# rbarile17/kelpie

Measured on AMD Instinct MI355X. Metric: candidate explanations evaluated/sec (incl. post-train) + rank-delta match rate, higher is better.
Workload: dtype bf16x3 (fp32-emulated)

## Files before the change

### kelpie_amd/csrc/kp_api.hip

```cpp
#include <cmath>
#include <cstdio>
#include <cstdlib>

#include "kp_common.hpp"
#include "kp_trace_check.hpp"

int cx_pick_db(int dim);

static thread_local std::string g_tls_err;

template <class F>
static int guarded(kp_ctx* c, F&& f) {
  try {
    f();
    if (c) c->err.clear();
    return KP_OK;
  } catch (const KpError& e) {
    if (c) c->err = e.msg;
    g_tls_err = e.msg;
    return e.code;
  } catch (const std::bad_alloc&) {
    if (c) c->err = "host out of memory";
    g_tls_err = "host out of memory";
    return KP_ENOMEM;
// ... 83 lines not shown
      KP_REQUIRE(m->model != KP_MODEL_COMPLEX || m->dim % 2 == 0, "ComplEx: row width must be even ([Re | Im])");
      int db = cx_pick_db(m->dim);
      KP_REQUIRE(db > 0, "row width > 400 not supported yet for ComplEx / ConvE");
      c->dp = 16 * db;
    } else if (m->model == KP_MODEL_DISTMULT) {
      int db = cx_pick_db(m->dim);
      if (db <= 0) throw KpError{KP_ENOTSUP, "DistMult: row width > 400 not supported"};
      c->dp = 16 * db;
    } else {
      c->dp = round_up(m->dim, 16);
    }
    c->attn_mode = 1;
    if (const char* a = std::getenv("KP_ATTN")) c->attn_mode = std::strcmp(a, "f32") == 0 ? 0 : 1;
    c->cv_fused = 1;
    if (const char* a = std::getenv("KP_CV_FUSED")) c->cv_fused = std::atoi(a) != 0;
    c->cv_shared = 1;
    if (const char* a = std::getenv("KP_CV_SHARED")) c->cv_shared = std::atoi(a) != 0;
    if (const char* a = std::getenv("KP_CV_RANK")) c->cv_rank64 = std::strcmp(a, "f32") != 0;
    if (const char* a = std::getenv("KP_CV_DX")) c->cv_dx_block = std::strcmp(a, "block") == 0;
    if (const char* a = std::getenv("KP_TE_RANK")) c->te_rank64 = std::strcmp(a, "f32") != 0;
    if (const char* a = std::getenv("KP_ATTN_PART"))
      c->attn_part = std::strcmp(a, "streamk") == 0 ? 1 : std::strcmp(a, "ranges") == 0 ? 2 : 0;
    if (const char* a = std::getenv("KP_ATTN_RANGES")) c->attn_ranges = std::max(0, std::min(16, std::atoi(a)));
    KP_HIP(hipStreamCreateWithFlags(&c->stream, hipStreamNonBlocking));
    {
      hipMemPool_t pool = device_pool(device);
      for (DevBuf* d : c->buffers()) {
        d->s = c->stream;
        d->pool = pool;
      }
    }
    KP_HIP(hipEventCreate(&c->ev0));
    KP_HIP(hipEventCreate(&c->ev1));
    upload_padded(c, &c->dE, m->entity, m->n_ent, m->dim, c->dp);
    upload_padded(c, &c->dR, m->relation, m->n_rel2, m->dim, c->dp);
    if (m->model == KP_MODEL_CONVE) {
      KP_REQUIRE(m->conv_w && m->conv_b && m->fc_w && m->fc_b && m->bn_alpha && m->bn_beta,
                 "ConvE: missing frozen layers");
      KP_REQUIRE(m->dim % 20 == 0 && m->dim / 20 >= 3, "ConvE: dim must be 20*h with h >= 3");
      c->hidden = 32 * 38 * (m->dim / 20 - 2);
      upload_plain(&c->d_conv_w, m->conv_w, 32 * 9);
      upload_plain(&c->d_conv_b, m->conv_b, 32);
      upload_plain(&c->d_fc_w, m->fc_w, (size_t)m->dim * c->hidden);
      upload_plain(&c->d_fc_b, m->fc_b, m->dim);
      upload_plain(&c->d_bn_a, m->bn_alpha, 1 + 32 + m->dim);
      upload_plain(&c->d_bn_b, m->bn_beta, 1 + 32 + m->dim);
// ... 315 lines not shown
```

### kelpie_amd/csrc/kp_attn3.hpp

```cpp
#pragma once
#include <type_traits>

#include "kp_attn.hpp"

#ifdef KP_ATTN3_STAMPS
#ifndef KP_DIAGNOSTIC_BUILD
#error "KP_ATTN3_STAMPS is a diagnostic build (make diag / tools/attn_micro.sh)"
#endif
__device__ unsigned long long g_attn3_stamps[8];
#define KP3_STAMP(v) v = __builtin_amdgcn_s_memtime()
#define KP3_ACC(i, a, b) st_acc[i] += (b) - (a)
#else
#define KP3_STAMP(v) (void)0
#define KP3_ACC(i, a, b) (void)0
#endif

#ifdef KP_ATTN3_CLOCK
#ifndef KP_DIAGNOSTIC_BUILD
#error "KP_ATTN3_CLOCK is a diagnostic build (tools/attn_micro.sh)"
#endif
__device__ unsigned long long g_attn3_clock[4096][4];
#endif

#ifndef KP_O_AHEAD
#define KP_O_AHEAD 1
#endif
#ifndef KP_S_AHEAD
#define KP_S_AHEAD 1
#endif
static_assert(KP_S_AHEAD >= 1 && KP_S_AHEAD <= 2, "KP_S_AHEAD: 1..2 (lgkmcnt holds at most 15)");
#if (defined(KP_DIAG_NO_S) || defined(KP_DIAG_NO_O) || defined(KP_ATTN_NODMA) || defined(KP_DIAG_DMA_LGKM0) || \
     defined(KP_DMA_SPREAD_ALL) || defined(KP_DIAG_S4) || defined(KP_DIAG_DMA_VM0) || defined(KP_DIAG_M0SAVE) || defined(KP_DIAG_NO_OSTORE) || defined(KP_DIAG_EARLY_EXIT) || defined(KP_DIAG_O_HALF) || defined(KP_DIAG_S_HALF) || defined(KP_DIAG_XTILE_W)) && \
// ... 145 lines not shown
  return c;
}

template <int DP>
__global__ void kp_split3_table(const float* __restrict__ E, int n_ent, uint8_t* __restrict__ out) {
  const long long i = (long long)blockIdx.x * blockDim.x + threadIdx.x;
  if (i >= (long long)n_ent * (DP / 2)) return;
  const int e = (int)(i / (DP / 2)), d = 2 * (int)(i % (DP / 2));
  __bf16 h[2], m[2], l[2];
  split3(E[(size_t)e * DP + d], h[0], m[0], l[0]);
  split3(E[(size_t)e * DP + d + 1], h[1], m[1], l[1]);
  __bf16* row = reinterpret_cast<__bf16*>(out + (size_t)e * split3_row_bytes(DP));
  row[d] = h[0];
  row[d + 1] = h[1];
  row[DP + d] = m[0];
  row[DP + d + 1] = m[1];
  row[2 * DP + d] = l[0];
  row[2 * DP + d + 1] = l[1];
}

template <int DB, int MODE>
constexpr int attn3_min_wgs() { return (MODE == ATT_BCE_O && 2 * attn3_lds_bytes(DB) <= 163840) ? 2 : 1; }

template <int DB, int MODE>
__global__ __launch_bounds__(256, (attn3_min_wgs<DB, MODE>())) void kp_attn3(const uint8_t* __restrict__ E3, int n_ent,
                                                   const float* __restrict__ Qpre, int nq, AttnWork wk,
                                                   float* __restrict__ out_m, float* __restrict__ out_l,
                                                   float* __restrict__ out_O, const float* __restrict__ qscale,
                                                   float ylo, const double* __restrict__ colpre) {
  constexpr bool WITH_O = MODE != ATT_SOFTMAX;
  constexpr int DP = 16 * DB;
  constexpr bool ASM = attn3_asm(DB);
  constexpr bool ILV = ASM && KP_ILV;
  constexpr int NK = DP / 32;
  constexpr int TAIL = (DP % 32) / 16;
  constexpr int KT = 32;
  constexpr int PART_B = 2 * DP;
  constexpr int ROW_B = split3_row_bytes(DP);
  constexpr bool BUFDMA = attn3_bufdma(DB);
  constexpr int PIECES = attn3_buf_pieces(DB);
  constexpr int BUF_B = 1024 * PIECES;
  extern __shared__ __attribute__((aligned(16))) uint8_t lds3[];

  const int tid = threadIdx.x;
#ifdef KP_DIAG_EARLY_EXIT
  if (ylo != 12345.f) return;
#endif
  if constexpr (KP_ATTN_PRIO > 0) __builtin_amdgcn_s_setprio(KP_ATTN_PRIO);
  const int lane = tid & 63;
  const int w = __builtin_amdgcn_readfirstlane(tid >> 6);
  const int g = lane >> 4, c = lane & 15;
  int key_begin = 0, key_end = 0;
  const uint32_t lds0 = (uint32_t)(uintptr_t)(__attribute__((address_space(3))) uint8_t*)lds3;
#ifdef KP_ATTN3_STAMPS
  unsigned long long st0 = 0, st1 = 0, st2 = 0, st3 = 0, st4 = 0;
  unsigned long long st_acc[5] = {0, 0, 0, 0, 0};
#endif

  const __amdgpu_buffer_rsrc_t e3rsrc = __builtin_amdgcn_make_buffer_rsrc(
      const_cast<uint8_t*>(E3), (short)0, (int)((n_ent + 31) / 32 * 32 * ROW_B + 1024), 0x00020000);
#if KP_O_SC1
  const __amdgpu_buffer_rsrc_t orsrc =
      __builtin_amdgcn_make_buffer_rsrc(out_O, (short)0, 0x7FFFFFFF, 0x00020000);
#endif
  auto bdma = [&](int tile, int buf, int p) {
    __builtin_amdgcn_raw_ptr_buffer_load_lds(
        e3rsrc, (__attribute__((address_space(3))) void*)(uintptr_t)(lds0 + (uint32_t)(buf * BUF_B + 1024 * p)), 16,
        16 * lane, (key_begin + tile * KT) * ROW_B + 1024 * p, 0, 0);
  };
  typedef int i32x4_t __attribute__((ext_vector_type(4)));
  const i32x4_t e3rs = {(int)(uint32_t)(uintptr_t)E3,
                        (int)(uint32_t)((uintptr_t)E3 >> 32) & 0xFFFF,
                        (int)((n_ent + 31) / 32 * 32 * ROW_B + 1024), 0x00020000};
  auto dma_group = [&](int tile, int buf, int g) {
    const int pb = w * ((PIECES + 3) / 4) + 4 * g;
    const uint32_t m0v = (uint32_t)__builtin_amdgcn_readfirstlane((int)(lds0 + (uint32_t)(buf * BUF_B + 1024 * pb)));
    const uint32_t so = (uint32_t)__builtin_amdgcn_readfirstlane((key_begin + tile * KT) * ROW_B + 1024 * pb);
    const int nleft = (PIECES + 3) / 4 - 4 * g;
    uint32_t keep;
// ... 82 lines not shown
  for (;;) {
    int qt, kt0, kt1, part;
    bool fill_rest;
    if (wk.ranges) {
      if (unit >= n_units) break;
      qt = unit % QT;
      part = unit / QT;
      kt0 = (int)((long long)part * wk.ktq / wk.ranges);
      kt1 = (int)((long long)(part + 1) * wk.ktq / wk.ranges);
      fill_rest = false;
      unit += (int)gridDim.x;
    } else {
      if (it >= it_end) break;
      qt = (int)(it / wk.ktq);
      kt0 = (int)(it - (long long)qt * wk.ktq);
      kt1 = (int)min((long long)wk.ktq, (long long)kt0 + (it_end - it));
      part = (int)blockIdx.x - (int)(((long long)qt * wk.ktq) / wk.per_wg);
      fill_rest = kt1 == wk.ktq;
      it += kt1 - kt0;
    }
    key_begin = kt0 * KT;
    key_end = min(n_ent, kt1 * KT);
    const int ntiles = kt1 - kt0;
    const int q = qt * 64 + 16 * w + c;
    const bool valid = q < nq;
    bf16x8 qb[NK > 0 ? NK : 1][3];
    bf16x4 qt4[3];
    float gsc = 0.f;
    if (MODE == ATT_BCE_O) gsc = valid ? qscale[q] : 0.f;
    {
      const float* qp = Qpre + (size_t)(valid ? q : 0) * DP;
#pragma unroll
      for (int s = 0; s < NK; ++s) {
        const float4 v0 = *reinterpret_cast<const float4*>(qp + 32 * s + 8 * g);
        const float4 v1 = *reinterpret_cast<const float4*>(qp + 32 * s + 8 * g + 4);
        const float f[8] = {v0.x, v0.y, v0.z, v0.w, v1.x, v1.y, v1.z, v1.w};
#pragma unroll
        for (int j = 0; j < 8; ++j) {
          __bf16 h, m, l;
          split3(valid ? f[j] : 0.f, h, m, l);
          qb[s][0][j] = h;
          qb[s][1][j] = m;
          qb[s][2][j] = l;
        }
      }
      if (TAIL) {
        const float4 v0 = *reinterpret_cast<const float4*>(qp + 32 * NK + 4 * g);
        const float f[4] = {v0.x, v0.y, v0.z, v0.w};
#pragma unroll
        for (int j = 0; j < 4; ++j) {
          __bf16 h, m, l;
          split3(valid ? f[j] : 0.f, h, m, l);
          qt4[0][j] = h;
          qt4[1][j] = m;
          qt4[2][j] = l;
        }
      }
    }
    f32x4 O[WITH_O ? DB : 1];
    float m_ref = kNegInf, l_run = 0.f;
    float csh = 0.f;

    for (int pass = 0; pass < 2; ++pass) {
#pragma unroll
      for (int j = 0; j < (WITH_O ? DB : 1); ++j) O[j] = (f32x4){0.f, 0.f, 0.f, 0.f};
      l_run = 0.f;
      float m_seen = kNegInf;
      if (ntiles > 0) issue(0, 0);
      asm volatile("s_waitcnt vmcnt(0)" ::: "memory");
      __syncthreads();
#ifdef KP_DIAG_XTILE_W
      float scp[2][4] = {{0.f, 0.f, 0.f, 0.f}, {0.f, 0.f, 0.f, 0.f}};
      float pwn[8] = {0.f, 0.f, 0.f, 0.f, 0.f, 0.f, 0.f, 0.f};
      float lacc = 0.f;
      bf16x8 pbn[3];
      float dtmp[8], htmp[8];
      auto wpiece = [&](int q) {
        if (q < 24) {
          const int j = q / 3, st = q % 3;
          if (st == 0) {
            dtmp[j] = scp[j >> 2][j & 3] - m_ref;
            m_seen = fmaxf(m_seen, scp[j >> 2][j & 3]);
          } else if (st == 1) {
            pwn[j] = __expf(dtmp[j]);
          } else {
            pwn[j] = __fsub_rn(pwn[j], csh);
            lacc += pwn[j];
          }
        } else if (q < 48) {
          const int j = (q - 24) / 3, st = (q - 24) % 3;
          if (st == 0) {
            const __bf16 h = (__bf16)pwn[j];
            pbn[0][j] = h;
// ... 333 lines not shown
        }
        KP3_STAMP(st3);
        asm volatile("s_waitcnt vmcnt(0)" ::: "memory");
        __syncthreads();
        KP3_STAMP(st4);
        KP3_ACC(0, st0, st1);
        KP3_ACC(1, st1, st2);
        KP3_ACC(2, st2, st3);
        KP3_ACC(3, st3, st4);
#ifdef KP_ATTN3_STAMPS
        st_acc[4] += 1;
#endif
      }
      if (MODE == ATT_BCE_O) break;
      float mq = fmaxf(m_seen, __shfl_xor(m_seen, 16, 64));
      mq = fmaxf(mq, __shfl_xor(mq, 32, 64));
#if defined(KP_DIAG_NO_S) || defined(KP_DIAG_NO_O)
      break;
#endif
      if (pass == 1 || !__syncthreads_or(mq > m_ref + kMargin)) break;
      m_ref = mq;
    }

    float l_tot = l_run + __shfl_xor(l_run, 16, 64);
    l_tot += __shfl_xor(l_tot, 32, 64);
    if (ntiles > 0) {
      l_tot = __fmaf_rn(csh, (float)(key_end - key_begin), l_tot);
      if (WITH_O) {
        const double* p0 = colpre + (size_t)kt0 * DP;
        const double* p1 = colpre + (size_t)kt1 * DP;
#pragma unroll
        for (int m = 0; m < DB; ++m) {
          const int d = 16 * m + 4 * g;
          const double2 a0 = *reinterpret_cast<const double2*>(p0 + d), a1 = *reinterpret_cast<const double2*>(p0 + d + 2);
          const double2 b0 = *reinterpret_cast<const double2*>(p1 + d), b1 = *reinterpret_cast<const double2*>(p1 + d + 2);
          O[m][0] = __fmaf_rn(csh, (float)(b0.x - a0.x), O[m][0]);
          O[m][1] = __fmaf_rn(csh, (float)(b0.y - a0.y), O[m][1]);
          O[m][2] = __fmaf_rn(csh, (float)(b1.x - a1.x), O[m][2]);
          O[m][3] = __fmaf_rn(csh, (float)(b1.y - a1.y), O[m][3]);
        }
      }
    }
    if (valid) {
      const size_t o = (size_t)part * nq + q;
      if (g == 0 && MODE != ATT_BCE_O) {
        out_m[o] = m_ref;
        out_l[o] = l_tot;
      }
#ifdef KP_DIAG_NO_OSTORE
      if (false) {
#else
// ... 7 lines not shown
          __builtin_amdgcn_raw_buffer_store_b128(__builtin_bit_cast(u32x4_t, O[m]), orsrc,
                                                 (int)((o * DP + 16 * m + 4 * g) * sizeof(float)), 0, 16);
#elif KP_O_NT
          __builtin_nontemporal_store(O[m], reinterpret_cast<f32x4*>(dst + 16 * m + 4 * g));
#else
          *reinterpret_cast<float4*>(dst + 16 * m + 4 * g) = make_float4(O[m][0], O[m][1], O[m][2], O[m][3]);
#endif
        }
      }
    }
    if (fill_rest && valid) {
      for (int pp = part + 1; pp < wk.n_parts; ++pp) {
        const size_t o = (size_t)pp * nq + q;
        if (g == 0 && MODE != ATT_BCE_O) {
          out_m[o] = kNegInf;
          out_l[o] = 0.f;
        }
        if (WITH_O) {
          float* dst = out_O + o * DP;
          for (int d = 4 * g; d < DP; d += 16) *reinterpret_cast<float4*>(dst + d) = make_float4(0.f, 0.f, 0.f, 0.f);
        }
      }
    }
  }
#ifdef KP_ATTN3_STAMPS
  if (lane == 0)
    for (int i = 0; i < 5; ++i) atomicAdd(&g_attn3_stamps[i], st_acc[i]);
#endif
#ifdef KP_ATTN3_CLOCK
  {
    unsigned long long ck_t1, ck_r1;
    asm volatile("s_waitcnt vmcnt(0)\n\ts_memtime %0\n\ts_memrealtime %1\n\ts_waitcnt lgkmcnt(0)"
                 : "=s"(ck_t1), "=s"(ck_r1)::"memory");
    if (tid == 0 && blockIdx.x < 4096) {
      g_attn3_clock[blockIdx.x][0] = ck_t0;
      g_attn3_clock[blockIdx.x][1] = ck_r0;
      g_attn3_clock[blockIdx.x][2] = ck_t1;
      g_attn3_clock[blockIdx.x][3] = ck_r1;
    }
  }
#endif
}

template <int DB>
const uint8_t* split3_image(kp_ctx* c) {
  constexpr int DP = 16 * DB;
  KP_REQUIRE(c->dp == DP, "attn3: table stride mismatch");
  if (!c->e3_ready) {
    const size_t n_pad = (size_t)(c->n_ent + 31) / 32 * 32;
    const size_t bytes = n_pad * split3_row_bytes(DP) + 1024;
// ... 23 lines not shown
  if (d >= DP) return;
  double s = 0.0;
  pre[d] = 0.0;
  for (int t = 0; t < ntiles; ++t) {
    s += ts[(size_t)t * DP + d];
    pre[(size_t)(t + 1) * DP + d] = s;
  }
}
template <int DB>
const double* tile_prefix(kp_ctx* c) {
  constexpr int DP = 16 * DB;
  if (!c->e3pre_ready) {
    const int ntiles = (c->n_ent + 31) / 32;
    double* ts = reinterpret_cast<double*>(c->e3ts.ensure(sizeof(double) * (size_t)ntiles * DP));
    double* pre = reinterpret_cast<double*>(c->e3pre.ensure(sizeof(double) * (size_t)(ntiles + 1) * DP));
    hipLaunchKernelGGL((kp_tile_sums<DP>), dim3((unsigned)ntiles), dim3((DP + 63) / 64 * 64), 0, c->stream, c->dE,
                       c->n_ent, ts);
    KP_HIP(hipGetLastError());
    hipLaunchKernelGGL((kp_tile_prefix<DP>), dim3((DP + 63) / 64), dim3(64), 0, c->stream, ts, ntiles, pre);
    KP_HIP(hipGetLastError());
    c->e3pre_ready = true;
  }
  return c->e3pre.as<double>();
}

template <int DB, int MODE = ATT_SOFTMAX_O>
int attn3_wpc(kp_ctx* c) {
  static_assert(MODE == ATT_SOFTMAX_O || MODE == ATT_BCE_O, "attn3_wpc: the launched O mode");
  int& slot = c->attn3_wpc[MODE == ATT_BCE_O ? 1 : 0];
  if (slot <= 0) {
    int n = 0;
    KP_HIP(hipOccupancyMaxActiveBlocksPerMultiprocessor(&n, kp_attn3<DB, MODE>, 256, attn3_lds_bytes(DB)));
    slot = std::max(1, n);
  }
  return slot;
}

#define KP_DB_CASE(N, DB_MIN, ...)   \
  case N:                            \
    if constexpr (N >= (DB_MIN)) {   \
      constexpr int DB = N;          \
      __VA_ARGS__;                   \
    }                                \
    break;
#define KP_DB_DISPATCH(DBV, DB_MIN, MSG, ...)      \
  switch ((DBV) >= (DB_MIN) ? (DBV) : -1) {        \
// ... 7 lines not shown
    default: throw KpError{KP_ENOTSUP, MSG};       \
  }

#ifndef KP_CV_ATTN_INFLIGHT
#define KP_CV_ATTN_INFLIGHT 0
#endif

inline AttnPlan attn_plan_ctx(const kp_ctx* c, int nq, int n_ent, int slots, bool inflight_ok) {
  if (c->attn_mode != 1) return attn_plan(nq, n_ent, slots);
  return attn_plan_select(c->attn_part, inflight_ok ? c->attn_inflight : 1, c->attn_ranges, nq, n_ent, slots);
}

inline void attn_plan_note(kp_ctx* c, const AttnPlan& p, int nq, bool inflight_ok) {
  if (nq < c->attn_last.nq) return;
  c->attn_last.nq = nq;
  c->attn_last.inflight = (c->attn_mode == 1 && inflight_ok) ? c->attn_inflight : 1;
  c->attn_last.ranges = p.wk.ranges;
  c->attn_last.n_parts = p.wk.n_parts;
  c->attn_last.n_wg = p.n_wg;
}

template <int DB, int MODE>
void launch_attn3(kp_ctx* c, int n_ent, const float* Q, int nq, const AttnPlan& plan, float* m, float* l, float* O,
                  const float* qscale, float ylo) {
  KP_REQUIRE(n_ent == c->n_ent, "attn3: key count differs from the table's (tile prefix sums)");
  KP_REQUIRE((long long)(n_ent + 31) / 32 * 32 * split3_row_bytes(16 * DB) + 1024 < (1LL << 31),
             "attn3: table too large for the 32-bit buffer descriptor of the split image");
  const uint8_t* E3 = split3_image<DB>(c);
  const double* pre = tile_prefix<DB>(c);
  hipLaunchKernelGGL((kp_attn3<DB, MODE>), dim3(plan.n_wg), dim3(256), attn3_lds_bytes(DB), c->stream, E3, n_ent, Q,
                     nq, plan.wk, m, l, O, qscale, ylo, pre);
  KP_HIP(hipGetLastError());
}

}
```

### kelpie_amd/csrc/kp_common.hpp

```cpp
#pragma once

#include <hip/hip_runtime.h>

#include <algorithm>
#include <array>
#include <cstdint>
#include <cstring>
#include <mutex>
#include <string>
#include <tuple>
#include <utility>
#include <vector>

#include "../../include/kelpie_hip.h"

typedef float f32x4 __attribute__((ext_vector_type(4)));

#define KP_WAVE 64

struct KpError {
  int code;
  std::string msg;
};

// ... 75 lines not shown
  DevBuf cand_key, cand_col;
  DevBuf top_ids, top_scores;
  DevBuf p_trip, p_po, p_filt_off, p_filt;
  DevBuf p_target, p_rank;
  DevBuf p_q64, p_t64, p_bits;
  auto all() {
    return std::array{&pred,     &po,       &filt_off, &filt,       &target,     &rank,   &q64,
                      &t64,      &scores,   &bits,     &cand_key,   &cand_col,   &top_ids, &top_scores,
                      &p_trip,   &p_po,     &p_filt_off, &p_filt,   &p_target,   &p_rank, &p_q64,
                      &p_t64,    &p_bits};
  }
};
KP_WS_COMPLETE(RankWs);

struct ComplexWs {
  DevBuf x, s1, s2;
  DevBuf plans, queries, targets;
  DevBuf pairs, acts;
  DevBuf stepq, stept;
  DevBuf contrib;
  DevBuf tsum, qpair, lsef;
  DevBuf am, al, ao;
  DevBuf qs;
  DevBuf score_q, score_out;
  DevBuf tr_term, tr_fe, tr_fr, tr_off, tr_loss;
  auto all() {
    return std::array{&x, &s1, &s2, &plans, &queries, &targets, &pairs, &acts, &stepq, &stept, &contrib,
                      &tsum, &qpair, &lsef, &am, &al, &ao, &qs, &score_q, &score_out, &tr_term, &tr_fe, &tr_fr,
                      &tr_off, &tr_loss};
  }
};
KP_WS_COMPLETE(ComplexWs);

struct TranseWs {
  DevBuf x;
  DevBuf slots, rows, rng;
  DevBuf order;
  DevBuf heads, rels;
  DevBuf tr_off, tr_loss;
  auto all() { return std::array{&x, &slots, &rows, &rng, &order, &heads, &rels, &tr_off, &tr_loss}; }
};
KP_WS_COMPLETE(TranseWs);

struct ConveWs {
  DevBuf x, s1, s2;
  DevBuf kinst, finst, acts;
  DevBuf tails;
  DevBuf keep_bits;
  DevBuf fcf, fpairs;
  DevBuf flat;
  DevBuf slab;
// ... 40 lines not shown
  int n_ent = 0, n_rel2 = 0, dim = 0, dp = 0;
  int hidden = 0;
  float* dE = nullptr;
  float* dR = nullptr;
  float* d_conv_w = nullptr;
  float* d_conv_b = nullptr;
  float* d_fc_w = nullptr;
  float* d_fc_wt = nullptr;
  float* d_fc_b = nullptr;
  float* d_bn_a = nullptr;
  float* d_bn_b = nullptr;
  std::vector<float> hE;
  RankWs rank;
  ComplexWs cx;
  TranseWs te;
  ConveWs cv;
  std::string err;
  Timing timing;
  bool time_hot = true;
  int attn_mode = 0;
  int attn_part = 0;
  int attn_inflight = 1;
  int attn_ranges = 0;
  struct AttnLast {
    int nq = -1, inflight = 1, ranges = 0, n_parts = 0, n_wg = 0;
  } attn_last;
  bool e3_ready = false;
  bool e3pre_ready = false;
  bool eT_ready = false;
  int cv_fused = 1;
  int cv_rank64 = 1;
  int cv_dx_block = 0;
  int te_norm = 2;
  int te_rank64 = 1;
  bool cvf_ready = false;
  int cv_shared = 1;
  bool cv_shared_ready = false;
  int attn3_wpc[2] = {0, 0};
  kp_train_state* train = nullptr;
  kp_cv_train* cvtrain = nullptr;
  std::vector<hipEvent_t> evpool;
  std::vector<std::pair<double, double>> hot_pairs;
  std::vector<double> hot_iv;
  std::vector<DevBuf*> buffers() {
    std::vector<DevBuf*> v;
    auto add = [&v](auto list) { v.insert(v.end(), list.begin(), list.end()); };
// ... 122 lines not shown
```

### kelpie_amd/csrc/kp_complex.hip

```cpp
#include <algorithm>
#include <cstdio>
#include <cstdlib>
#include <cmath>

#include "kp_attn.hpp"
#include "kp_attn3.hpp"
#include "kp_cx_plan.hpp"
#include "kp_posttrain.hpp"

namespace {
using namespace kpattn;

__device__ __forceinline__ double cx_q64(const float* __restrict__ lhs, const float* __restrict__ rel, int d,
                                         int half) {
  if (d < half) return (double)lhs[d] * (double)rel[d] - (double)lhs[d + half] * (double)rel[d + half];
  if (d < 2 * half) {
    const int i = d - half;
    return (double)lhs[i] * (double)rel[d] + (double)lhs[d] * (double)rel[i];
  }
  return 0.0;
}

struct CxProd {
  static constexpr int G = 2;
// ... 23 lines not shown

struct DmProd {
  static constexpr int G = 1;
  static constexpr const char* name = "DistMult";
  static int extent(int dim) { return dim; }
  static __device__ __forceinline__ float q(const float* __restrict__ lhs, const float* __restrict__ rel, int d,
                                            int w) {
    return d < w ? __fmul_rn(lhs[d], rel[d]) : 0.f;
  }
  static __device__ __forceinline__ double q64(const float* __restrict__ lhs, const float* __restrict__ rel, int d,
                                               int w) {
    return d < w ? (double)lhs[d] * (double)rel[d] : 0.0;
  }
  static __device__ __forceinline__ float mod(const float* xv) { return fabsf(xv[0]); }
  static __device__ __forceinline__ double mod64(const float* xv) { return fabs((double)xv[0]); }
  static __device__ __forceinline__ void emit(float* __restrict__ out, int i, int w, const double* xv,
                                              const double* rv, const double* dv, double cf) {
    const double q = xv[0] * rv[0];
    out[i] = (float)(dv[0] * rv[0] + cf * q);
  }
};

template <class Prod>
__global__ void kp_cx_qpair(const float* __restrict__ E, const float* __restrict__ R, int dp, int half,
                            const int2* __restrict__ pairs, int n_pairs, float* __restrict__ out) {
  int p = blockIdx.x;
  if (p >= n_pairs) return;
  int2 hr = pairs[p];
  const float* lhs = E + (size_t)hr.x * dp;
  const float* rel = R + (size_t)hr.y * dp;
  for (int d = threadIdx.x; d < dp; d += blockDim.x) out[(size_t)p * dp + d] = Prod::q(lhs, rel, d, half);
}

__global__ void kp_cx_lse_merge(int npairs, int n_split, const float* __restrict__ am, const float* __restrict__ al,
                                float* __restrict__ lsef) {
  const int p = blockIdx.x * blockDim.x + threadIdx.x;
  if (p >= npairs) return;
  float mm = kNegInf;
  for (int s = 0; s < n_split; ++s) mm = fmaxf(mm, am[(size_t)s * npairs + p]);
  double ll = 0.0;
  for (int s = 0; s < n_split; ++s) {
    const float ms = am[(size_t)s * npairs + p];
    if (ms != kNegInf) ll += (double)al[(size_t)s * npairs + p] * exp((double)ms - (double)mm);
  }
  lsef[p] = (float)((double)mm + log(ll));
}

__global__ void kp_cx_tsum(const float* __restrict__ E, int dp, const CxQuery* __restrict__ pq, int nq,
                           const int32_t* __restrict__ targets, float* __restrict__ tsum) {
  int q = blockIdx.x;
  if (q >= nq) return;
  CxQuery Q = pq[q];
  for (int d = threadIdx.x; d < dp; d += blockDim.x) {
    float acc = 0.f;
// ... 381 lines not shown
      const float* eo = E + (size_t)o * DP;
      for (int d = 0; d < DP; ++d) t = __fma_rn(q[d], (double)eo[d], t);
    } else {
      t = z;
    }
    kcol64[s] = z;
    t64[s] = t;
  }
}

template <class Prod>
__global__ void kp_cx_scoreq(const float* __restrict__ E, const float* __restrict__ R, int dp, int half,
                             const int32_t* __restrict__ heads, const int32_t* __restrict__ rels, int n,
                             float* __restrict__ Q) {
  int s = blockIdx.x;
  if (s >= n) return;
  const float* lhs = E + (size_t)heads[s] * dp;
  const float* rel = R + (size_t)rels[s] * dp;
  for (int d = threadIdx.x; d < dp; d += blockDim.x) Q[(size_t)s * dp + d] = Prod::q(lhs, rel, d, half);
}

template <int DP, class Prod>
__global__ void kp_cx_stepq(const float* __restrict__ X, const float* __restrict__ R, int half,
                            const int4* __restrict__ stepq, int nq, float* __restrict__ Q) {
  const int j = blockIdx.x;
  if (j >= nq) return;
  const int4 sq = stepq[j];
  const float* x = X + (size_t)sq.x * DP;
  const float* rel = R + (size_t)sq.y * DP;
  for (int d = threadIdx.x; d < DP; d += blockDim.x) Q[(size_t)j * DP + d] = Prod::q(x, rel, d, half);
}

template <int DB, class Prod>
void launch_stepq(kp_ctx* c, const int4* stepq, const float* X, int nq, float* Q) {
  if (nq <= 0) return;
  hipLaunchKernelGGL((kp_cx_stepq<16 * DB, Prod>), dim3(nq), dim3(64), 0, c->stream, X, c->dR, Prod::extent(c->dim), stepq,
                     nq, Q);
  KP_HIP(hipGetLastError());
}

template <int DB>
int attn_slots_db(kp_ctx* c) {
  if (c->attn_mode == 1) return c->n_cu * attn3_wpc<DB>(c);
  return c->n_cu * (DB <= 13 ? 2 : 1);
}

template <int DB>
void launch_attn(kp_ctx* c, bool with_o, const float* Q, int nq, const AttnPlan& plan, float* m, float* l,
                 float* O) {
  if (nq <= 0) return;
  if (c->attn_mode == 1) {
    if (with_o)
      launch_attn3<DB, ATT_SOFTMAX_O>(c, c->n_ent, Q, nq, plan, m, l, O, nullptr, 0.f);
    else
      launch_attn3<DB, ATT_SOFTMAX>(c, c->n_ent, Q, nq, plan, m, l, O, nullptr, 0.f);
    return;
  }
  const size_t shm = attn_lds_bytes(DB);
  if (with_o)
    hipLaunchKernelGGL((kp_attn<DB, ATT_SOFTMAX_O>), dim3(plan.n_wg), dim3(256), shm, c->stream, c->dE, c->n_ent, Q,
                       nq, plan.wk, m, l, O, nullptr, 0.f);
  else
    hipLaunchKernelGGL((kp_attn<DB, ATT_SOFTMAX>), dim3(plan.n_wg), dim3(256), shm, c->stream, c->dE, c->n_ent, Q,
                       nq, plan.wk, m, l, O, nullptr, 0.f);
  KP_HIP(hipGetLastError());
}

struct CxTraceDev {
  double *term = nullptr, *freg_e = nullptr, *freg_r = nullptr;
  const int32_t* targets = nullptr;
  const int2* pairs = nullptr;
  int32_t* off = nullptr;
  float* loss = nullptr;
  int total = 0;
};

template <int DB, class Prod>
void launch_update(kp_ctx* c, int n_act, const int4* act, const CxPlan* plans, const CxQuery* pq,
// ... 53 lines not shown
  opt.one_minus_b1 = (float)(1.0 - (double)hp->beta1);
  opt.one_minus_b2 = (float)(1.0 - (double)hp->beta2);
  opt.reg_w = hp->reg_weight;
  KP_REQUIRE(hp->reg_kind == KP_REG_N3 || hp->reg_kind == KP_REG_N2, who + ": unknown regulariser");
  opt.reg_n2 = hp->reg_kind == KP_REG_N2;
  return opt;
}

struct CxDev {
  float *X, *S1, *S2;
  CxPlan* plans;
  CxQuery* pq;
  int32_t* tg;
  int2* pairs;
  int4 *acts, *stepq, *stept;
  float *contrib, *tsum, *qpair, *lsef;
  Rank64Dev r64;
  int32_t* pred;
  RankDev rk;
  ProbeDev probes;
  CxTraceDev trace;
  float *am = nullptr, *al = nullptr, *ao = nullptr, *qs = nullptr;
  std::vector<AttnPlan> step_plan;
};

static_assert(sizeof(CxI2) == sizeof(int2) && alignof(CxI2) == alignof(int2), "CxI2 is int2");
static_assert(sizeof(CxI4) == sizeof(int4) && alignof(CxI4) == alignof(int4), "CxI4 is int4");
inline const int2* as_dev(const CxI2* p) { return reinterpret_cast<const int2*>(p); }
inline const int4* as_dev(const CxI4* p) { return reinterpret_cast<const int4*>(p); }

CxDev cx_workspaces(kp_ctx* c, const kp_batch* bt, const TopkOut& tk, const CxStepPlan& sp, std::vector<float>& xp) {
  const int ns = bt->n_slots, DP = c->dp;
  CxDev d;
  d.X = upload_x0(c, c->cx.x, bt, xp);
  d.S1 = reinterpret_cast<float*>(c->cx.s1.ensure(sizeof(float) * (size_t)ns * DP));
  d.S2 = reinterpret_cast<float*>(c->cx.s2.ensure(sizeof(float) * (size_t)ns * DP));
  KP_HIP(hipMemsetAsync(d.S1, 0, sizeof(float) * (size_t)ns * DP, c->stream));
  KP_HIP(hipMemsetAsync(d.S2, 0, sizeof(float) * (size_t)ns * DP, c->stream));
  d.plans = upload(c, c->cx.plans, sp.plans.data(), sp.plans.size());
  d.pq = upload(c, c->cx.queries, sp.pqs.data(), sp.pqs.size());
  d.tg = upload(c, c->cx.targets, sp.targets.data(), sp.targets.size());
  d.pairs = upload(c, c->cx.pairs, as_dev(sp.pairs.data()), sp.pairs.size());
  d.acts = upload(c, c->cx.acts, as_dev(sp.acts.data()), sp.acts.size());
  d.stepq = upload(c, c->cx.stepq, as_dev(sp.stepq.data()), sp.stepq.size());
  d.stept = upload(c, c->cx.stept, as_dev(sp.stept.data()), sp.stept.size());
  d.contrib = reinterpret_cast<float*>(c->cx.contrib.ensure(sizeof(float) * (size_t)std::max(1, sp.max_items) * DP));
// ... 35 lines not shown
                       reg_n2, d.trace.freg_e);
    KP_HIP(hipGetLastError());
    hipLaunchKernelGGL(kp_cx_rowreg<Prod>, dim3((c->n_rel2 + 3) / 4), dim3(256), 0, c->stream, c->dR, c->n_rel2, DP,
                       half, reg_n2, d.trace.freg_r);
    KP_HIP(hipGetLastError());
  }
  int slots_attn = 0;
  CX_DISPATCH(DBV, slots_attn = attn_slots_db<DB>(c));
  const AttnPlan plan_pairs = attn_plan_ctx(c, std::max(npairs, 1), c->n_ent, slots_attn, true);
  const int split_pairs = plan_pairs.wk.n_parts;
  size_t att_rows = (size_t)std::max(npairs, 1) * split_pairs;
  d.step_plan.resize(sp.T);
  c->attn_last = {};
  for (int t = 0; t < sp.T; ++t) {
    const int nq = sp.q_off[t + 1] - sp.q_off[t];
    d.step_plan[t] = attn_plan_ctx(c, std::max(nq, 1), c->n_ent, slots_attn, true);
    if (nq > 0) attn_plan_note(c, d.step_plan[t], nq, true);
    att_rows = std::max(att_rows, (size_t)nq * d.step_plan[t].wk.n_parts);
  }
  d.am = reinterpret_cast<float*>(c->cx.am.ensure(sizeof(float) * att_rows));
  d.al = reinterpret_cast<float*>(c->cx.al.ensure(sizeof(float) * att_rows));
  d.ao = reinterpret_cast<float*>(c->cx.ao.ensure(sizeof(float) * att_rows * DP));
  d.qs = reinterpret_cast<float*>(c->cx.qs.ensure(sizeof(float) * (size_t)std::max(sp.max_nq, 1) * DP));
  if (npairs > 0) {
    hipLaunchKernelGGL(kp_cx_qpair<Prod>, dim3(npairs), dim3(128), 0, c->stream, c->dE, c->dR, DP, Prod::extent(c->dim),
                       d.pairs, npairs, d.qpair);
    KP_HIP(hipGetLastError());
    CX_DISPATCH(DBV, launch_attn<DB>(c, false, d.qpair, npairs, plan_pairs, d.am, d.al, nullptr));
    hipLaunchKernelGGL(kp_cx_lse_merge, dim3((npairs + 255) / 256), dim3(256), 0, c->stream, npairs, split_pairs, d.am,
                       d.al, d.lsef);
    KP_HIP(hipGetLastError());
  }
}

template <class Prod>
int64_t cx_step_loop(kp_ctx* c, const kp_hp* hp, const CxStepPlan& sp, const CxDev& d, CxOpt opt, double* t_steps) {
  const int DBV = c->dp / 16, T = sp.T;
  int64_t hot_launches = 0;
  c->hot_pairs.clear();
  c->hot_iv.clear();
  for (int t = 0; t < T; ++t) {
    const int nq = sp.q_off[t + 1] - sp.q_off[t];
    const int na = sp.act_off[t + 1] - sp.act_off[t];
    const int sp_n = d.step_plan[t].wk.n_parts;
    hipEvent_t ea = nullptr, eb = nullptr;
    if (nq > 0 && c->time_hot) {
      ea = c->event(2 * hot_launches);
      eb = c->event(2 * hot_launches + 1);
    }
    CX_DISPATCH(DBV, launch_stepq<DB, Prod>(c, d.stepq + sp.q_off[t], d.X, nq, d.qs));
    if (nq > 0 && c->time_hot) KP_HIP(hipEventRecord(ea, c->stream));
    CX_DISPATCH(DBV, launch_attn<DB>(c, true, d.qs, nq, d.step_plan[t], d.am, d.al, d.ao));
    if (nq > 0) {
      if (c->time_hot) {
        KP_HIP(hipEventRecord(eb, c->stream));
        c->hot_pairs.push_back({(double)nq, 0.0});
      }
      ++hot_launches;
    }
    const AdamStep as = adam_step(hp, t);
    opt.step_size = as.step_size;
    opt.bc2_sqrt = as.bc2_sqrt;
    CX_DISPATCH(DBV, launch_update<DB, Prod>(c, na, d.acts + sp.act_off[t], d.plans, d.pq, d.stepq + sp.q_off[t], nq,
                                             d.stept + sp.t_off[t], sp.t_off[t + 1] - sp.t_off[t], d.tsum, d.qpair,
                                             d.lsef, d.am, d.al, d.ao, sp_n, d.contrib, d.X, d.S1, d.S2, opt,
                                             d.trace, t));
    if (g_host_times) {
      if (t == 0) t_steps[0] = host_ms();
      if (t == 1) t_steps[1] = host_ms();
      if (t == T / 2) t_steps[2] = host_ms();
      if (t == T - 1) t_steps[3] = host_ms();
    }
  }
  return hot_launches;
}
// ... 110 lines not shown
```

Measured before the change: 997.5.

## Issue first key tile before query split and precompute range column sums

By default (attn_ends=1) the attention kernel now loads the query floats and issues the first key-tile DMA before splitting the query into three bf16 parts, so the split overlaps the load. It also uses per-range column-sum deltas precomputed once in fp32, replacing per-unit double prefix reads. An optional mode (KP_ATTN_QIMG) makes the stepq and qpair kernels write a pre-split query image in fragment layout, so the attention kernel loads bf16 fragments directly. The costs are an extra small kernel launch, extra buffers, fp32 instead of double column sums, and padded query kernel grids.

```diff
diff --git a/kelpie_amd/csrc/kp_api.hip b/kelpie_amd/csrc/kp_api.hip
--- a/kelpie_amd/csrc/kp_api.hip
+++ b/kelpie_amd/csrc/kp_api.hip
@@ -129,6 +129,7 @@
     if (const char* a = std::getenv("KP_ATTN_PART"))
       c->attn_part = std::strcmp(a, "streamk") == 0 ? 1 : std::strcmp(a, "ranges") == 0 ? 2 : 0;
     if (const char* a = std::getenv("KP_ATTN_RANGES")) c->attn_ranges = std::max(0, std::min(16, std::atoi(a)));
+    if (const char* a = std::getenv("KP_ATTN_QIMG")) c->attn_ends = std::atoi(a) != 0 ? 2 : 0;
     KP_HIP(hipStreamCreateWithFlags(&c->stream, hipStreamNonBlocking));
     {
       hipMemPool_t pool = device_pool(device);
diff --git a/kelpie_amd/csrc/kp_attn3.hpp b/kelpie_amd/csrc/kp_attn3.hpp
--- a/kelpie_amd/csrc/kp_attn3.hpp
+++ b/kelpie_amd/csrc/kp_attn3.hpp
@@ -2,12 +2,13 @@
 #include <type_traits>
 
 #include "kp_attn.hpp"
+#include "kp_attn_qimg.hpp"
 
 #ifdef KP_ATTN3_STAMPS
 #ifndef KP_DIAGNOSTIC_BUILD
 #error "KP_ATTN3_STAMPS is a diagnostic build (make diag / tools/attn_micro.sh)"
 #endif
-__device__ unsigned long long g_attn3_stamps[8];
+__device__ unsigned long long g_attn3_stamps[12];
 #define KP3_STAMP(v) v = __builtin_amdgcn_s_memtime()
 #define KP3_ACC(i, a, b) st_acc[i] += (b) - (a)
 #else
@@ -199,13 +200,15 @@
 template <int DB, int MODE>
 constexpr int attn3_min_wgs() { return (MODE == ATT_BCE_O && 2 * attn3_lds_bytes(DB) <= 163840) ? 2 : 1; }
 
-template <int DB, int MODE>
+template <int DB, int MODE, int ENDS = 0>
 __global__ __launch_bounds__(256, (attn3_min_wgs<DB, MODE>())) void kp_attn3(const uint8_t* __restrict__ E3, int n_ent,
                                                    const float* __restrict__ Qpre, int nq, AttnWork wk,
                                                    float* __restrict__ out_m, float* __restrict__ out_l,
                                                    float* __restrict__ out_O, const float* __restrict__ qscale,
-                                                   float ylo, const double* __restrict__ colpre) {
+                                                   float ylo, const double* __restrict__ colpre,
+                                                   const uint8_t* __restrict__ Qimg, const float* __restrict__ dcol) {
   constexpr bool WITH_O = MODE != ATT_SOFTMAX;
+  constexpr bool QIMG = ENDS == 2, EARLY = ENDS >= 1;
   constexpr int DP = 16 * DB;
   constexpr bool ASM = attn3_asm(DB);
   constexpr bool ILV = ASM && KP_ILV;
@@ -231,7 +234,8 @@
   const uint32_t lds0 = (uint32_t)(uintptr_t)(__attribute__((address_space(3))) uint8_t*)lds3;
 #ifdef KP_ATTN3_STAMPS
   unsigned long long st0 = 0, st1 = 0, st2 = 0, st3 = 0, st4 = 0;
-  unsigned long long st_acc[5] = {0, 0, 0, 0, 0};
+  unsigned long long st_acc[9] = {0, 0, 0, 0, 0, 0, 0, 0, 0};
+  unsigned long long su0 = 0, su1 = 0, su2 = 0, su3 = 0;
 #endif
 
   const __amdgpu_buffer_rsrc_t e3rsrc = __builtin_amdgcn_make_buffer_rsrc(
@@ -360,18 +364,47 @@
     key_begin = kt0 * KT;
     key_end = min(n_ent, kt1 * KT);
     const int ntiles = kt1 - kt0;
+    KP3_STAMP(su0);
     const int q = qt * 64 + 16 * w + c;
     const bool valid = q < nq;
     bf16x8 qb[NK > 0 ? NK : 1][3];
     bf16x4 qt4[3];
     float gsc = 0.f;
     if (MODE == ATT_BCE_O) gsc = valid ? qscale[q] : 0.f;
-    {
+    if constexpr (QIMG) {
+      if (ntiles > 0) issue(0, 0);
+      const uint8_t* qi = Qimg + qimg_frag_off(DP, qt, w, 0, 0, lane);
+#pragma unroll
+      for (int s = 0; s < NK; ++s)
+#pragma unroll
+        for (int p = 0; p < 3; ++p)
+          qb[s][p] = *reinterpret_cast<const bf16x8*>(qi + (3 * s + p) * qimg_frag_bytes(false));
+      if (TAIL) {
+#pragma unroll
+        for (int p = 0; p < 3; ++p)
+          qt4[p] = *reinterpret_cast<const bf16x4*>(Qimg + qimg_frag_off(DP, qt, w, NK, p, lane));
+      }
+#pragma unroll
+      for (int s = 0; s < NK; ++s)
+#pragma unroll
+        for (int p = 0; p < 3; ++p) asm volatile("" : "+v"(qb[s][p]));
+      if (TAIL) {
+#pragma unroll
+        for (int p = 0; p < 3; ++p) asm volatile("" : "+v"(qt4[p]));
+      }
+    } else if constexpr (EARLY) {
       const float* qp = Qpre + (size_t)(valid ? q : 0) * DP;
+      float4 fv[NK > 0 ? NK : 1][2], ft = make_float4(0.f, 0.f, 0.f, 0.f);
 #pragma unroll
       for (int s = 0; s < NK; ++s) {
-        const float4 v0 = *reinterpret_cast<const float4*>(qp + 32 * s + 8 * g);
-        const float4 v1 = *reinterpret_cast<const float4*>(qp + 32 * s + 8 * g + 4);
+        fv[s][0] = *reinterpret_cast<const float4*>(qp + 32 * s + 8 * g);
+        fv[s][1] = *reinterpret_cast<const float4*>(qp + 32 * s + 8 * g + 4);
+      }
+      if (TAIL) ft = *reinterpret_cast<const float4*>(qp + 32 * NK + 4 * g);
+      if (ntiles > 0) issue(0, 0);
+#pragma unroll
+      for (int s = 0; s < NK; ++s) {
+        const float4 v0 = fv[s][0], v1 = fv[s][1];
         const float f[8] = {v0.x, v0.y, v0.z, v0.w, v1.x, v1.y, v1.z, v1.w};
 #pragma unroll
         for (int j = 0; j < 8; ++j) {
@@ -383,7 +416,7 @@
         }
       }
       if (TAIL) {
-        const float4 v0 = *reinterpret_cast<const float4*>(qp + 32 * NK + 4 * g);
+        const float4 v0 = ft;
         const float f[4] = {v0.x, v0.y, v0.z, v0.w};
 #pragma unroll
         for (int j = 0; j < 4; ++j) {
@@ -394,6 +427,34 @@
           qt4[2][j] = l;
         }
       }
+    } else {
+      const float* qp = Qpre + (size_t)(valid ? q : 0) * DP;
+#pragma unroll
+      for (int s = 0; s < NK; ++s) {
+        const float4 v0 = *reinterpret_cast<const float4*>(qp + 32 * s + 8 * g);
+        const float4 v1 = *reinterpret_cast<const float4*>(qp + 32 * s + 8 * g + 4);
+        const float f[8] = {v0.x, v0.y, v0.z, v0.w, v1.x, v1.y, v1.z, v1.w};
+#pragma unroll
+        for (int j = 0; j < 8; ++j) {
+          __bf16 h, m, l;
+          split3(valid ? f[j] : 0.f, h, m, l);
+          qb[s][0][j] = h;
+          qb[s][1][j] = m;
+          qb[s][2][j] = l;
+        }
+      }
+      if (TAIL) {
+        const float4 v0 = *reinterpret_cast<const float4*>(qp + 32 * NK + 4 * g);
+        const float f[4] = {v0.x, v0.y, v0.z, v0.w};
+#pragma unroll
+        for (int j = 0; j < 4; ++j) {
+          __bf16 h, m, l;
+          split3(valid ? f[j] : 0.f, h, m, l);
+          qt4[0][j] = h;
+          qt4[1][j] = m;
+          qt4[2][j] = l;
+        }
+      }
     }
     f32x4 O[WITH_O ? DB : 1];
     float m_ref = kNegInf, l_run = 0.f;
@@ -404,9 +465,12 @@
       for (int j = 0; j < (WITH_O ? DB : 1); ++j) O[j] = (f32x4){0.f, 0.f, 0.f, 0.f};
       l_run = 0.f;
       float m_seen = kNegInf;
-      if (ntiles > 0) issue(0, 0);
+      if (ntiles > 0 && !(EARLY && pass == 0)) issue(0, 0);
       asm volatile("s_waitcnt vmcnt(0)" ::: "memory");
       __syncthreads();
+#ifdef KP_ATTN3_STAMPS
+      if (pass == 0) KP3_STAMP(su1);
+#endif
 #ifdef KP_DIAG_XTILE_W
       float scp[2][4] = {{0.f, 0.f, 0.f, 0.f}, {0.f, 0.f, 0.f, 0.f}};
       float pwn[8] = {0.f, 0.f, 0.f, 0.f, 0.f, 0.f, 0.f, 0.f};
@@ -786,11 +850,22 @@
       m_ref = mq;
     }
 
+    KP3_STAMP(su2);
     float l_tot = l_run + __shfl_xor(l_run, 16, 64);
     l_tot += __shfl_xor(l_tot, 32, 64);
     if (ntiles > 0) {
       l_tot = __fmaf_rn(csh, (float)(key_end - key_begin), l_tot);
-      if (WITH_O) {
+      if (WITH_O && EARLY && dcol != nullptr) {
+        const float* dc = dcol + (size_t)part * DP + 4 * g;
+#pragma unroll
+        for (int m = 0; m < DB; ++m) {
+          const float4 dv = *reinterpret_cast<const float4*>(dc + 16 * m);
+          O[m][0] = __fmaf_rn(csh, dv.x, O[m][0]);
+          O[m][1] = __fmaf_rn(csh, dv.y, O[m][1]);
+          O[m][2] = __fmaf_rn(csh, dv.z, O[m][2]);
+          O[m][3] = __fmaf_rn(csh, dv.w, O[m][3]);
+        }
+      } else if (WITH_O) {
         const double* p0 = colpre + (size_t)kt0 * DP;
         const double* p1 = colpre + (size_t)kt1 * DP;
 #pragma unroll
@@ -844,10 +919,20 @@
         }
       }
     }
+#ifdef KP_ATTN3_STAMPS
+    asm volatile("s_waitcnt vmcnt(0)" ::: "memory");
+    KP3_STAMP(su3);
+    if (ntiles > 0) {
+      KP3_ACC(5, su0, su1);
+      KP3_ACC(6, su1, su2);
+      KP3_ACC(7, su2, su3);
+      st_acc[8] += 1;
+    }
+#endif
   }
 #ifdef KP_ATTN3_STAMPS
   if (lane == 0)
-    for (int i = 0; i < 5; ++i) atomicAdd(&g_attn3_stamps[i], st_acc[i]);
+    for (int i = 0; i < 9; ++i) atomicAdd(&g_attn3_stamps[i], st_acc[i]);
 #endif
 #ifdef KP_ATTN3_CLOCK
   {
@@ -917,6 +1002,24 @@
     c->e3pre_ready = true;
   }
   return c->e3pre.as<double>();
+}
+
+template <int DP>
+__global__ void kp_attn3_dcol(const double* __restrict__ colpre, int ktq, int ranges, float* __restrict__ dcol) {
+  const int i = blockIdx.x * blockDim.x + threadIdx.x;
+  if (i >= ranges * DP) return;
+  const int part = i / DP, d = i % DP;
+  const int kt0 = (int)((long long)part * ktq / ranges);
+  const int kt1 = (int)((long long)(part + 1) * ktq / ranges);
+  dcol[i] = (float)(colpre[(size_t)kt1 * DP + d] - colpre[(size_t)kt0 * DP + d]);
+}
+template <int DB>
+void launch_attn3_dcol(kp_ctx* c, const AttnWork& wk, float* dcol) {
+  constexpr int DP = 16 * DB;
+  const double* pre = tile_prefix<DB>(c);
+  hipLaunchKernelGGL((kp_attn3_dcol<DP>), dim3((wk.ranges * DP + 255) / 256), dim3(256), 0, c->stream, pre, wk.ktq,
+                     wk.ranges, dcol);
+  KP_HIP(hipGetLastError());
 }
 
 template <int DB, int MODE = ATT_SOFTMAX_O>
@@ -970,14 +1073,30 @@
 
 template <int DB, int MODE>
 void launch_attn3(kp_ctx* c, int n_ent, const float* Q, int nq, const AttnPlan& plan, float* m, float* l, float* O,
-                  const float* qscale, float ylo) {
+                  const float* qscale, float ylo, int ends = 0, const uint8_t* qimg = nullptr,
+                  const float* dcol = nullptr) {
   KP_REQUIRE(n_ent == c->n_ent, "attn3: key count differs from the table's (tile prefix sums)");
   KP_REQUIRE((long long)(n_ent + 31) / 32 * 32 * split3_row_bytes(16 * DB) + 1024 < (1LL << 31),
              "attn3: table too large for the 32-bit buffer descriptor of the split image");
   const uint8_t* E3 = split3_image<DB>(c);
   const double* pre = tile_prefix<DB>(c);
+  if constexpr (MODE != ATT_BCE_O) {
+    if (ends != 0) {
+      KP_REQUIRE((ends == 1 && !qimg) || (ends == 2 && qimg), "attn3: the query image belongs to form 2");
+      KP_REQUIRE(!dcol || plan.wk.ranges > 0, "attn3: range column sums with a stream-K plan");
+      if (ends == 2)
+        hipLaunchKernelGGL((kp_attn3<DB, MODE, 2>), dim3(plan.n_wg), dim3(256), attn3_lds_bytes(DB), c->stream, E3,
+                           n_ent, Q, nq, plan.wk, m, l, O, qscale, ylo, pre, qimg, dcol);
+      else
+        hipLaunchKernelGGL((kp_attn3<DB, MODE, 1>), dim3(plan.n_wg), dim3(256), attn3_lds_bytes(DB), c->stream, E3,
+                           n_ent, Q, nq, plan.wk, m, l, O, qscale, ylo, pre, qimg, dcol);
+      KP_HIP(hipGetLastError());
+      return;
+    }
+  }
+  KP_REQUIRE(ends == 0 && !qimg && !dcol, "attn3: this launch has form 0 of the units' ends only");
   hipLaunchKernelGGL((kp_attn3<DB, MODE>), dim3(plan.n_wg), dim3(256), attn3_lds_bytes(DB), c->stream, E3, n_ent, Q,
-                     nq, plan.wk, m, l, O, qscale, ylo, pre);
+                     nq, plan.wk, m, l, O, qscale, ylo, pre, (const uint8_t*)nullptr, (const float*)nullptr);
   KP_HIP(hipGetLastError());
 }
 
diff --git a/kelpie_amd/csrc/kp_attn_qimg.hpp b/kelpie_amd/csrc/kp_attn_qimg.hpp
--- /dev/null
+++ b/kelpie_amd/csrc/kp_attn_qimg.hpp
@@ -0,0 +1,39 @@
+#pragma once
+#include <cstddef>
+
+#if defined(__HIPCC__)
+#define KP_QIMG_FN __host__ __device__ constexpr
+#else
+#define KP_QIMG_FN constexpr
+#endif
+
+namespace kpattn {
+
+KP_QIMG_FN int qimg_nk(int DP) { return DP / 32; }
+KP_QIMG_FN int qimg_tail(int DP) { return (DP % 32) / 16; }
+KP_QIMG_FN int qimg_frag_bytes(bool tail) { return tail ? 64 * 8 : 64 * 16; }
+KP_QIMG_FN int qimg_wave_bytes(int DP) {
+  return 3 * (qimg_nk(DP) * qimg_frag_bytes(false) + qimg_tail(DP) * qimg_frag_bytes(true));
+}
+KP_QIMG_FN int qimg_tile_bytes(int DP) { return 4 * qimg_wave_bytes(DP); }
+KP_QIMG_FN size_t qimg_bytes(int DP, int nq) { return (size_t)((nq + 63) / 64) * (size_t)qimg_tile_bytes(DP); }
+
+KP_QIMG_FN size_t qimg_frag_off(int DP, int qt, int w, int s, int p, int lane) {
+  const int nk = qimg_nk(DP);
+  const int in_wave = s < nk ? (3 * s + p) * qimg_frag_bytes(false) + 16 * lane
+                             : 3 * nk * qimg_frag_bytes(false) + p * qimg_frag_bytes(true) + 8 * lane;
+  return (size_t)qt * (size_t)qimg_tile_bytes(DP) + (size_t)(w * qimg_wave_bytes(DP) + in_wave);
+}
+
+KP_QIMG_FN int qimg_row_items(int DP) { return 4 * (qimg_nk(DP) + qimg_tail(DP)); }
+KP_QIMG_FN int qimg_item_dim0(int DP, int i) {
+  return i < 4 * qimg_nk(DP) ? 8 * i : 32 * qimg_nk(DP) + 4 * (i - 4 * qimg_nk(DP));
+}
+KP_QIMG_FN int qimg_item_dims(int DP, int i) { return i < 4 * qimg_nk(DP) ? 8 : 4; }
+KP_QIMG_FN size_t qimg_item_off(int DP, int q, int i, int p) {
+  const int nk = qimg_nk(DP);
+  const int s = i < 4 * nk ? i / 4 : nk, g = i < 4 * nk ? i % 4 : i - 4 * nk;
+  return qimg_frag_off(DP, q / 64, (q % 64) / 16, s, p, 16 * g + q % 16);
+}
+
+}
diff --git a/kelpie_amd/csrc/kp_common.hpp b/kelpie_amd/csrc/kp_common.hpp
--- a/kelpie_amd/csrc/kp_common.hpp
+++ b/kelpie_amd/csrc/kp_common.hpp
@@ -121,11 +121,13 @@
   DevBuf tsum, qpair, lsef;
   DevBuf am, al, ao;
   DevBuf qs;
+  DevBuf qs_img, qpair_img;
+  DevBuf dcol;
   DevBuf score_q, score_out;
   DevBuf tr_term, tr_fe, tr_fr, tr_off, tr_loss;
   auto all() {
     return std::array{&x, &s1, &s2, &plans, &queries, &targets, &pairs, &acts, &stepq, &stept, &contrib,
-                      &tsum, &qpair, &lsef, &am, &al, &ao, &qs, &score_q, &score_out, &tr_term, &tr_fe, &tr_fr,
+                      &tsum, &qpair, &lsef, &am, &al, &ao, &qs, &qs_img, &qpair_img, &dcol, &score_q, &score_out, &tr_term, &tr_fe, &tr_fr,
                       &tr_off, &tr_loss};
   }
 };
@@ -212,6 +214,7 @@
   int attn_part = 0;
   int attn_inflight = 1;
   int attn_ranges = 0;
+  int attn_ends = 1;
   struct AttnLast {
     int nq = -1, inflight = 1, ranges = 0, n_parts = 0, n_wg = 0;
   } attn_last;
diff --git a/kelpie_amd/csrc/kp_complex.hip b/kelpie_amd/csrc/kp_complex.hip
--- a/kelpie_amd/csrc/kp_complex.hip
+++ b/kelpie_amd/csrc/kp_complex.hip
@@ -69,14 +69,53 @@
 };
 
 template <class Prod>
+__device__ __forceinline__ void cx_qimg_row(uint8_t* __restrict__ img, int dp, int j, bool live,
+                                            const float* __restrict__ lhs, const float* __restrict__ rel, int half) {
+  const int items = qimg_row_items(dp);
+  for (int i = threadIdx.x; i < items; i += blockDim.x) {
+    const int d0 = qimg_item_dim0(dp, i);
+    if (qimg_item_dims(dp, i) == 8) {
+      bf16x8 pc[3];
+#pragma unroll
+      for (int k = 0; k < 8; ++k) {
+        __bf16 h, m, l;
+        split3(live ? Prod::q(lhs, rel, d0 + k, half) : 0.f, h, m, l);
+        pc[0][k] = h;
+        pc[1][k] = m;
+        pc[2][k] = l;
+      }
+#pragma unroll
+      for (int p = 0; p < 3; ++p) *reinterpret_cast<bf16x8*>(img + qimg_item_off(dp, j, i, p)) = pc[p];
+    } else {
+      bf16x4 pc[3];
+#pragma unroll
+      for (int k = 0; k < 4; ++k) {
+        __bf16 h, m, l;
+        split3(live ? Prod::q(lhs, rel, d0 + k, half) : 0.f, h, m, l);
+        pc[0][k] = h;
+        pc[1][k] = m;
+        pc[2][k] = l;
+      }
+#pragma unroll
+      for (int p = 0; p < 3; ++p) *reinterpret_cast<bf16x4*>(img + qimg_item_off(dp, j, i, p)) = pc[p];
+    }
+  }
+}
+
+template <class Prod>
 __global__ void kp_cx_qpair(const float* __restrict__ E, const float* __restrict__ R, int dp, int half,
-                            const int2* __restrict__ pairs, int n_pairs, float* __restrict__ out) {
+                            const int2* __restrict__ pairs, int n_pairs, float* __restrict__ out,
+                            uint8_t* __restrict__ img) {
   int p = blockIdx.x;
-  if (p >= n_pairs) return;
+  if (p >= n_pairs) {
+    if (img) cx_qimg_row<Prod>(img, dp, p, false, nullptr, nullptr, half);
+    return;
+  }
   int2 hr = pairs[p];
   const float* lhs = E + (size_t)hr.x * dp;
   const float* rel = R + (size_t)hr.y * dp;
   for (int d = threadIdx.x; d < dp; d += blockDim.x) out[(size_t)p * dp + d] = Prod::q(lhs, rel, d, half);
+  if (img) cx_qimg_row<Prod>(img, dp, p, true, lhs, rel, half);
 }
 
 __global__ void kp_cx_lse_merge(int npairs, int n_split, const float* __restrict__ am, const float* __restrict__ al,
@@ -504,20 +543,26 @@
 
 template <int DP, class Prod>
 __global__ void kp_cx_stepq(const float* __restrict__ X, const float* __restrict__ R, int half,
-                            const int4* __restrict__ stepq, int nq, float* __restrict__ Q) {
+                            const int4* __restrict__ stepq, int nq, float* __restrict__ Q,
+                            uint8_t* __restrict__ img) {
   const int j = blockIdx.x;
-  if (j >= nq) return;
+  if (j >= nq) {
+    if (img) cx_qimg_row<Prod>(img, DP, j, false, nullptr, nullptr, half);
+    return;
+  }
   const int4 sq = stepq[j];
   const float* x = X + (size_t)sq.x * DP;
   const float* rel = R + (size_t)sq.y * DP;
   for (int d = threadIdx.x; d < DP; d += blockDim.x) Q[(size_t)j * DP + d] = Prod::q(x, rel, d, half);
+  if (img) cx_qimg_row<Prod>(img, DP, j, true, x, rel, half);
 }
 
 template <int DB, class Prod>
-void launch_stepq(kp_ctx* c, const int4* stepq, const float* X, int nq, float* Q) {
+void launch_stepq(kp_ctx* c, const int4* stepq, const float* X, int nq, float* Q, uint8_t* img) {
   if (nq <= 0) return;
-  hipLaunchKernelGGL((kp_cx_stepq<16 * DB, Prod>), dim3(nq), dim3(64), 0, c->stream, X, c->dR, Prod::extent(c->dim), stepq,
-                     nq, Q);
+  const int rows = img ? (nq + 63) / 64 * 64 : nq;
+  hipLaunchKernelGGL((kp_cx_stepq<16 * DB, Prod>), dim3(rows), dim3(64), 0, c->stream, X, c->dR, Prod::extent(c->dim),
+                     stepq, nq, Q, img);
   KP_HIP(hipGetLastError());
 }
 
@@ -529,13 +574,13 @@
 
 template <int DB>
 void launch_attn(kp_ctx* c, bool with_o, const float* Q, int nq, const AttnPlan& plan, float* m, float* l,
-                 float* O) {
+                 float* O, const uint8_t* qimg = nullptr, const float* dcol = nullptr) {
   if (nq <= 0) return;
   if (c->attn_mode == 1) {
     if (with_o)
-      launch_attn3<DB, ATT_SOFTMAX_O>(c, c->n_ent, Q, nq, plan, m, l, O, nullptr, 0.f);
+      launch_attn3<DB, ATT_SOFTMAX_O>(c, c->n_ent, Q, nq, plan, m, l, O, nullptr, 0.f, c->attn_ends, qimg, dcol);
     else
-      launch_attn3<DB, ATT_SOFTMAX>(c, c->n_ent, Q, nq, plan, m, l, O, nullptr, 0.f);
+      launch_attn3<DB, ATT_SOFTMAX>(c, c->n_ent, Q, nq, plan, m, l, O, nullptr, 0.f, c->attn_ends, qimg, nullptr);
     return;
   }
   const size_t shm = attn_lds_bytes(DB);
@@ -635,6 +680,8 @@
   CxTraceDev trace;
   float *am = nullptr, *al = nullptr, *ao = nullptr, *qs = nullptr;
   std::vector<AttnPlan> step_plan;
+  uint8_t *qs_img = nullptr, *qpair_img = nullptr;
+  std::vector<const float*> step_dcol;
 };
 
 static_assert(sizeof(CxI2) == sizeof(int2) && alignof(CxI2) == alignof(int2), "CxI2 is int2");
@@ -716,11 +763,38 @@
   d.al = reinterpret_cast<float*>(c->cx.al.ensure(sizeof(float) * att_rows));
   d.ao = reinterpret_cast<float*>(c->cx.ao.ensure(sizeof(float) * att_rows * DP));
   d.qs = reinterpret_cast<float*>(c->cx.qs.ensure(sizeof(float) * (size_t)std::max(sp.max_nq, 1) * DP));
+  d.step_dcol.assign(sp.T, nullptr);
+  if (c->attn_mode == 1 && c->attn_ends == 2) {
+    d.qs_img = reinterpret_cast<uint8_t*>(c->cx.qs_img.ensure(qimg_bytes(DP, std::max(sp.max_nq, 1))));
+    d.qpair_img = reinterpret_cast<uint8_t*>(c->cx.qpair_img.ensure(qimg_bytes(DP, std::max(npairs, 1))));
+  }
+  if (c->attn_mode == 1 && c->attn_ends >= 1) {
+    int dcol_off[17], dcol_rows = 0;
+    std::fill(dcol_off, dcol_off + 17, -1);
+    for (int t = 0; t < sp.T; ++t) {
+      const int S = d.step_plan[t].wk.ranges;
+      KP_REQUIRE(S >= 0 && S <= 16, "attn3: more ranges than the consumers merge");
+      if (S > 0 && sp.q_off[t + 1] > sp.q_off[t] && dcol_off[S] < 0) {
+        dcol_off[S] = dcol_rows;
+        dcol_rows += S;
+      }
+    }
+    float* dcol = reinterpret_cast<float*>(c->cx.dcol.ensure(sizeof(float) * (size_t)std::max(dcol_rows, 1) * DP));
+    for (int t = 0; t < sp.T; ++t) {
+      const int S = d.step_plan[t].wk.ranges;
+      if (S <= 0 || dcol_off[S] < 0 || sp.q_off[t + 1] <= sp.q_off[t]) continue;
+      float* at = dcol + (size_t)dcol_off[S] * DP;
+      if (std::find(d.step_dcol.begin(), d.step_dcol.begin() + t, at) == d.step_dcol.begin() + t)
+        CX_DISPATCH(DBV, launch_attn3_dcol<DB>(c, d.step_plan[t].wk, at));
+      d.step_dcol[t] = at;
+    }
+  }
   if (npairs > 0) {
-    hipLaunchKernelGGL(kp_cx_qpair<Prod>, dim3(npairs), dim3(128), 0, c->stream, c->dE, c->dR, DP, Prod::extent(c->dim),
-                       d.pairs, npairs, d.qpair);
+    const int pair_rows = d.qpair_img ? (npairs + 63) / 64 * 64 : npairs;
+    hipLaunchKernelGGL(kp_cx_qpair<Prod>, dim3(pair_rows), dim3(128), 0, c->stream, c->dE, c->dR, DP,
+                       Prod::extent(c->dim), d.pairs, npairs, d.qpair, d.qpair_img);
     KP_HIP(hipGetLastError());
-    CX_DISPATCH(DBV, launch_attn<DB>(c, false, d.qpair, npairs, plan_pairs, d.am, d.al, nullptr));
+    CX_DISPATCH(DBV, launch_attn<DB>(c, false, d.qpair, npairs, plan_pairs, d.am, d.al, nullptr, d.qpair_img));
     hipLaunchKernelGGL(kp_cx_lse_merge, dim3((npairs + 255) / 256), dim3(256), 0, c->stream, npairs, split_pairs, d.am,
                        d.al, d.lsef);
     KP_HIP(hipGetLastError());
@@ -742,9 +816,9 @@
       ea = c->event(2 * hot_launches);
       eb = c->event(2 * hot_launches + 1);
     }
-    CX_DISPATCH(DBV, launch_stepq<DB, Prod>(c, d.stepq + sp.q_off[t], d.X, nq, d.qs));
+    CX_DISPATCH(DBV, launch_stepq<DB, Prod>(c, d.stepq + sp.q_off[t], d.X, nq, d.qs, d.qs_img));
     if (nq > 0 && c->time_hot) KP_HIP(hipEventRecord(ea, c->stream));
-    CX_DISPATCH(DBV, launch_attn<DB>(c, true, d.qs, nq, d.step_plan[t], d.am, d.al, d.ao));
+    CX_DISPATCH(DBV, launch_attn<DB>(c, true, d.qs, nq, d.step_plan[t], d.am, d.al, d.ao, d.qs_img, d.step_dcol[t]));
     if (nq > 0) {
       if (c->time_hot) {
         KP_HIP(hipEventRecord(eb, c->stream));
```

After: 1007 (median of 6 runs). Within noise of the previous version (+1.0%).
